# HMS-IDAC/UnMicst

Measured on AMD Instinct MI355X. Metric: tiles/sec (256x256x2) whole-slide inference, higher is better.
Workload: dtype f16x3, cross terms of the layers at <= 1/4 resolution as block-scaled fp6 (MX e2m3) MFMA products; fp32 accumulate

## Files before the change

### unmicst_amd/csrc/umx_conv_f16.hip

```cpp
#include <type_traits>

#include "umx_kernels.h"

namespace umx {

typedef _Float16 h8 __attribute__((ext_vector_type(8)));
typedef float f32x4 __attribute__((ext_vector_type(4)));

template <int I> struct IC { static constexpr int value = I; };
template <int B, int E, typename F>
__device__ __forceinline__ void static_for(F&& f) {
    if constexpr (B < E) {
        f(IC<B>{});
        static_for<B + 1, E>(f);
    }
}

#define UMX_GLDS16(gptr, lptr)                                                                        \
    __builtin_amdgcn_global_load_lds((const __attribute__((address_space(1))) void*)(gptr),           \
                                     (__attribute__((address_space(3))) void*)(lptr), 16, 0, 0)

typedef int i32x6 __attribute__((ext_vector_type(6)));
typedef int i32x8 __attribute__((ext_vector_type(8)));
typedef _Float16 h32 __attribute__((ext_vector_type(32)));

typedef unsigned u32x16 __attribute__((ext_vector_type(16)));
#define UMX_MAX3(dst, a, b, c) asm volatile("v_pk_maximum3_f16 %0, %1, %2, %3" : "=v"(dst) : "v"(a), "v"(b), "v"(c))
#define UMX_MAX3N(dst, a, b, c) asm volatile("v_pk_maximum3_f16 %0, %1, %2, %3 neg_lo:[1,1,1] neg_hi:[1,1,1]" : "=v"(dst) : "v"(a), "v"(b), "v"(c))
#define UMX_MAX3N2(dst, a, b, c) asm volatile("v_pk_maximum3_f16 %0, %1, %2, %3 neg_lo:[0,0,1] neg_hi:[0,0,1]" : "=v"(dst) : "v"(a), "v"(b), "v"(c))
template <int NB>
__device__ __forceinline__ void quant_blocks_e2m3(const h8 (&v)[NB][4], i32x6 (&out)[NB], int (&scale_e8m0)[NB]) {
    h32 x[NB];
    u32x16 d[NB];
#pragma unroll
    for (int b = 0; b < NB; ++b) {
#pragma unroll
        for (int p = 0; p < 4; ++p)
#pragma unroll
            for (int j = 0; j < 8; ++j) x[b][8 * p + j] = v[b][p][j];
        d[b] = __builtin_bit_cast(u32x16, x[b]);
    }
    unsigned P[NB][5], N[NB][5];
#pragma unroll
    for (int t = 0; t < 5; ++t)
#pragma unroll
        for (int b = 0; b < NB; ++b) {
            UMX_MAX3(P[b][t], d[b][3 * t], d[b][3 * t + 1], d[b][3 * t + 2]);
            UMX_MAX3N(N[b][t], d[b][3 * t], d[b][3 * t + 1], d[b][3 * t + 2]);
        }
    unsigned P2[NB][2], N2[NB][2], m2[NB];
#pragma unroll
    for (int b = 0; b < NB; ++b) {
        UMX_MAX3(P2[b][0], P[b][0], P[b][1], P[b][2]);
        UMX_MAX3(N2[b][0], N[b][0], N[b][1], N[b][2]);
    }
#pragma unroll
    for (int b = 0; b < NB; ++b) {
        UMX_MAX3(P2[b][1], P[b][3], P[b][4], d[b][15]);
        UMX_MAX3N2(N2[b][1], N[b][3], N[b][4], d[b][15]);
    }
#pragma unroll
    for (int b = 0; b < NB; ++b) UMX_MAX3(m2[b], P2[b][0], P2[b][1], N2[b][0]);
#pragma unroll
    for (int b = 0; b < NB; ++b) UMX_MAX3(m2[b], m2[b], N2[b][1], N2[b][1]);
#pragma unroll
    for (int b = 0; b < NB; ++b) {
        const unsigned m = m2[b] & 0x7fff7fffu;
        const unsigned mm = max(m & 0xffffu, m >> 16);
        const unsigned ef = __float_as_uint((float)__builtin_bit_cast(_Float16, (unsigned short)mm)) >> 23;
        const unsigned e = max(ef, 3u) - 2u;
        scale_e8m0[b] = (int)e;
        const float sc = __uint_as_float(e << 23);
        asm volatile("v_cvt_scalef32_pk32_fp6_f16 %0, %1, %2" : "=&v"(out[b]) : "v"(x[b]), "v"(sc));
    }
}
__device__ __forceinline__ void quant_block_e2m3(const h8 (&v)[4], i32x6& out, int& scale_e8m0) {
    h8 vv[1][4] = {{v[0], v[1], v[2], v[3]}};
    i32x6 o[1];
    int s[1];
    quant_blocks_e2m3<1>(vv, o, s);
    out = o[0];
    scale_e8m0 = s[0];
}

constexpr int conv_f16x3_waves(int NT, int KMT, int NPH, int MAXP, bool D2S = false) {
    return NPH != 1 || D2S ? 2 : (NT <= 3 && MAXP == 4) ? 4 : (NT <= 3 || (NT <= 5 && MAXP == 4)) ? 3 : 2;
}
template <int NT, int KMT, int NPH, bool DBG = false, int MAXP = 4, bool PK = false, bool D2S = false, bool F6 = false, bool W2 = F6>
__global__ void __launch_bounds__(F6 ? 512 : 256, conv_f16x3_waves(NT, KMT, NPH, MAXP, D2S)) conv_f16x3(const HConvParams p) {
    static_assert(W2 == F6, "W2 only keeps the instantiation names stable: the two-tile workgroup is the F6 form");
    static_assert(!F6 || (NPH == 1 && !PK && !D2S && !DBG), "the fp6 cross-term form runs on the plain / per-phase kernel (no stamped twin: it spills 426 registers)");
    extern __shared__ __attribute__((aligned(16))) unsigned char smem[];

    const int tid = threadIdx.x;
    const int lane = tid & 63;
    constexpr int kNW = F6 ? 2 * kWaves : kWaves;
    const int wave_all = __builtin_amdgcn_readfirstlane(tid >> 6);
    const int half = F6 ? wave_all >> 2 : 0;
    const int wave = F6 ? wave_all & 3 : wave_all;
    const int q = lane >> 4;
    const int li = lane & 15;

    const int TWm = 1 << p.twm_log2, TH = 1 << p.th_log2;
    int bid = blockIdx.x, nblk_i = blockIdx.y, z_i = NPH == 1 ? blockIdx.z : 0;
    if (p.xcd_order == 2) {
        const int YZ = p.nblocks * (NPH == 1 ? p.nphase : 1);
        const int xcd = bid & 7, idx = bid >> 3;
        const int tl = idx / YZ, yz = idx - tl * YZ;
        const int q8 = p.ntiles_grid >> 3, r8 = p.ntiles_grid & 7;
        bid = xcd < r8 ? xcd * (q8 + 1) + tl : r8 * (q8 + 1) + (xcd - r8) * q8 + tl;
        nblk_i = yz % p.nblocks;
        z_i = yz / p.nblocks;
        if (tl >= (xcd < r8 ? q8 + 1 : q8)) return;
    } else if (p.xcd_order) {
        const int nb = gridDim.x, q8 = nb >> 3, r8 = nb & 7, xcd = bid & 7, idx = bid >> 3;
        bid = xcd < r8 ? xcd * (q8 + 1) + idx : r8 * (q8 + 1) + (xcd - r8) * q8 + idx;
    }
    if constexpr (F6) bid = 2 * bid + half;
    const int tx_i = bid % p.tiles_x; bid /= p.tiles_x;
    const int ty_i = bid % p.tiles_y; bid /= p.tiles_y;
    const int img0 = min(bid * p.imgs, p.B);
    const int y0 = ty_i * TH, x0 = tx_i * TWm;
    const HPhase& ph = p.ph[z_i];
    int ph_stage0 = ph.stage0, ph_nstages = ph.nstages;
    size_t split_off = 0;
    if (p.ksplit > 1) {
        const int ks = nblk_i / p.nblocks;
        nblk_i -= ks * p.nblocks;
        ph_stage0 += p.ks0[z_i][ks];
        ph_nstages = p.ks0[z_i][ks + 1] - p.ks0[z_i][ks];
        split_off = (size_t)ks * p.split_stride;
    }
    const int nblk = nblk_i;
    long long t_in = 0, t_wait = 0, t_comp = 0, t_a = 0, t_b = 0, t_vm = 0, t_iss = 0;
    if (DBG && p.dbg) t_in = __builtin_amdgcn_s_memtime();
    int abase[KMT];
#pragma unroll
    for (int m = 0; m < KMT; ++m) {
        const int t = wave * KMT + m;
        const int ig = t >> p.th_log2, ty = t & (TH - 1);
        abase[m] = ((ig * p.nimg_m + (li >> p.twm_log2)) * p.imgplane + ty * p.hw + (li & (TWm - 1))) * p.pix_bytes;
    }

    f32x4 accs[NPH][KMT][NT];
#pragma unroll
    for (int h = 0; h < NPH; ++h)
#pragma unroll
        for (int m = 0; m < KMT; ++m)
#pragma unroll
            for (int n = 0; n < NT; ++n) accs[h][m][n] = (f32x4){0.f, 0.f, 0.f, 0.f};

    const int lo_off = p.lo_off;
    unsigned char* const smem_h = smem + half * p.b_off;
    unsigned char* const Bl = smem + (F6 ? 2 : 1) * p.b_off;
    const uint4* const wbase = ph.w + (size_t)nblk * ph.wblk_stride;

    const int pl = (lane * p.inv_oc_q16) >> 16;
    const int kq = lane - pl * p.OC;
    int pix[MAXP];
#pragma unroll
    for (int j = 0; j < MAXP; ++j) {
        const int px = (wave + kWaves * j) * p.PP + pl;
        int v = -1;
        if (lane < p.nact && px < p.nhalo) {
            const int il = (int)(((float)px + 0.5f) * p.inv_imgplane);
            const int r = px - il * p.imgplane;
            const int hy = (int)(((float)r + 0.5f) * p.inv_hw);
            const int hx = r - hy * p.hw;
            const int gy = y0 + p.ymin + hy, gx = x0 + p.xmin + hx;
            const bool inside = img0 + il < p.B && gy >= 0 && gy < p.H && gx >= 0 && gx < p.W;
            v = inside ? (il * p.H + gy) * p.W + gx : -2;
        }
        pix[j] = v;
    }
    const size_t img_elems = (size_t)p.H * p.W;
    auto act_rsrc = [&](const _Float16* base, int Cs) {
        const size_t left = (size_t)(p.B - img0) * img_elems * Cs * 2;
        return __builtin_amdgcn_make_buffer_rsrc((void*)(base + (size_t)img0 * img_elems * Cs), 0,
                                                 (int)(left < 0x7fffffffu ? left : 0x7fffffffu), 0x00020000);
    };
    const __amdgpu_buffer_rsrc_t r0h = act_rsrc(p.src_hi[0], p.Cs[0]), r0l = act_rsrc(p.src_lo[0], p.Cs[0]);
    const __amdgpu_buffer_rsrc_t r1h = act_rsrc(p.src_hi[1] ? p.src_hi[1] : p.src_hi[0], p.Cs[1]),
                                 r1l = act_rsrc(p.src_lo[1] ? p.src_lo[1] : p.src_lo[0], p.Cs[1]);
    const __amdgpu_buffer_rsrc_t rw =
        __builtin_amdgcn_make_buffer_rsrc((void*)wbase, 0, ph.wblk_stride * 16, 0x00020000);
    const int lane16 = lane * 16;
#define UMX_BLDS16(rsrc, lptr, voff, soff) \
    __builtin_amdgcn_raw_ptr_buffer_load_lds(rsrc, (__attribute__((address_space(3))) void*)(lptr), 16, voff, soff, 0, 0)

    const int kqB0 = kq * p.srcB[0], kqB1 = kq * p.srcB[1];
    auto issue_halo = [&](const HStage& st) {
        const bool g1 = st.group > 0;
        const int pixA = p.srcA[g1 ? 1 : 0];
        const int kqB = g1 ? kqB1 : kqB0;
        const __amdgpu_buffer_rsrc_t rh = g1 ? r1h : r0h, rl = g1 ? r1l : r0l;
        unsigned char* const slot = smem_h + st.plane0 * p.slot_bytes;
        const int soff = st.oct0 * p.srcB[g1 ? 1 : 0];
        const bool kok = kq < st.noct;
#pragma unroll
        for (int j = 0; j < MAXP; ++j) {
            const int i = wave + kWaves * j;
            if (i >= p.ninst) break;
            int pj = pix[j];
            asm volatile("" : "+v"(pj));
            if (pj != -1 && kok) {
                const int voff = pj >= 0 ? (int)__umul24(pj, pixA) + kqB : 0x7fffffff;
                UMX_BLDS16(rh, slot + i * p.piece_bytes, voff, soff);
                UMX_BLDS16(rl, slot + lo_off + i * p.piece_bytes, voff, soff);
            }
        }
    };
    int wq_np = 0, wq_soff = 0;
    unsigned char* wq_dst = Bl;
    const int wq_w = wave_all * 1024;
    auto wq_begin = [&](const HStage& st, int buf) {
        unsigned char* const wl = Bl + buf * p.wbuf_bytes;
        if (wave_all == kNW - 1 && lane < 4) UMX_BLDS16(rw, wl, lane16, st.woff * 16);
        wq_np = F6 ? NT * 4096 : st.nk * (NT * 2048);
        wq_soff = st.woff * 16 + 64;
        wq_dst = wl + 64;
    };
    auto wq_one = [&](int c) {
        const int pc = wq_w + c * (kNW * 1024);
        if (pc < wq_np) UMX_BLDS16(rw, wq_dst + pc, lane16, wq_soff + pc);
    };
    auto wq_drain = [&](int c0) {
        for (int pc = wq_w + c0 * (kNW * 1024); pc < wq_np; pc += kNW * 1024)
            UMX_BLDS16(rw, wq_dst + pc, lane16, wq_soff + pc);
    };

    const int ec_units = (p.head_K > 0 ? (4 + p.head_K) * (NT * 4) + 4 : NT * 16) + (D2S ? 16 : 0);
    auto issue_econst = [&](int buf) {
        if (wave_all == kNW - 1) {
            float* const dst = reinterpret_cast<float*>(Bl + buf * p.wbuf_bytes);
#pragma unroll
            for (int i = 0; i < (8 * NT * 4 + 4 + 63) / 64; ++i)
                if (i * 64 + lane < ec_units)
                    UMX_GLDS16(p.econst + (size_t)nblk * ec_units + i * 64 + lane, dst + i * 256);
        }
    };
    auto issue_app = [&](int buf) {
        if constexpr (D2S) {
            if (p.app_c != nullptr && p.d2s_mix && wave == kWaves - 2) {
                const int apb = 4 * p.app_cw;
                const size_t oHW = (size_t)p.outH * p.outW, left = (size_t)(p.B - img0) * oHW * apb;
                const __amdgpu_buffer_rsrc_t ra = __builtin_amdgcn_make_buffer_rsrc(
                    (void*)(p.app_c + (size_t)img0 * oHW * apb), 0, (int)(left < 0x7fffffffu ? left : 0x7fffffffu), 0x00020000);
                unsigned char* const dst = Bl + buf * p.wbuf_bytes + ec_units * 16;
                const int oy = (lane >> 4) & 1, seg = lane & 15;
#pragma unroll
                for (int i = 0; i < kMW / 2; ++i) {
                    const int t = 2 * i + (lane >> 5);
                    const int irel = (t >> p.th_log2) * p.nimg_m, yt = y0 + (t & (TH - 1));
                    const bool ok = img0 + irel < p.B && seg * 16 < 32 * apb;
                    const int voff = ok ? (int)((irel * (int)oHW + (2 * yt + oy) * p.outW + 2 * x0) * apb + seg * 16) : 0x7fffffff;
                    UMX_BLDS16(ra, dst + i * 1024, voff, 0);
                }
            }
        }
    };
    const int par0 = (ph_nstages + 1) & 1;
    const float* const ec = reinterpret_cast<const float*>(Bl + p.wbuf_bytes);
    if (ph_nstages == 0) { issue_econst(1); issue_app(1); }
    typedef unsigned u32x4 __attribute__((ext_vector_type(4)));
    static_assert(sizeof(HStage) == 16, "one stage = one 16-byte scalar load");
    auto load_stage = [&](int idx) {
        const u32x4 raw = ((const __attribute__((address_space(4))) u32x4*)(unsigned long long)p.stages)[idx];
        HStage st;
        __builtin_memcpy(&st, &raw, sizeof(st));
        return st;
    };
    HStage cur = load_stage(ph_stage0);
    if (ph_nstages > 0) {
        if (cur.group >= 0) issue_halo(cur);
        wq_begin(cur, par0);
        wq_drain(0);
    }
    long long t_pro = 0;
    if (DBG && p.dbg) { t_pro = __builtin_amdgcn_s_memtime(); t_a = t_pro; }
    auto stage_body = [&](const int s) {
        const HStage nxt = load_stage(ph_stage0 + (s + 1 < ph_nstages ? s + 1 : s));
        asm volatile("s_waitcnt vmcnt(0)" ::: "memory");
        if (DBG && p.dbg) { const long long t_v = __builtin_amdgcn_s_memtime(); t_vm += t_v - t_a; }
        __syncthreads();
        if (DBG && p.dbg) { t_b = __builtin_amdgcn_s_memtime(); t_wait += t_b - t_a; }
        if (s + 1 < ph_nstages) {
            if (nxt.group >= 0) issue_halo(nxt);
            wq_begin(nxt, (s + 1 + par0) & 1);
        } else {
            wq_np = 0;
            issue_econst(1);
            issue_app(1);
        }
        if (DBG && p.dbg) t_iss += (long long)__builtin_amdgcn_s_memtime() - t_b;

        const unsigned char* const wl = Bl + ((s + par0) & 1) * p.wbuf_bytes;
        const int cur_nk = F6 ? (cur.nk & 0xff) : cur.nk;
        unsigned kbs[kStageK];
#pragma unroll
        for (int j = 0; j < (F6 ? 2 : kStageK); ++j)
            kbs[j] = (unsigned)*reinterpret_cast<const unsigned short*>(wl + (j * 4 + q) * 2) << 4;
        auto kstep = [&](int h, int j, bool sk) {
            constexpr int kLo = NT / 2, kHi = 2 * (NT / 2);
            constexpr int kImg = F6 ? 1024 : 2048;
            auto live = [&](int n) { return !(D2S && sk && n >= kLo && n < kHi); };
            const unsigned char* const bp = wl + 64 + j * (NT * kImg) + lane * 16;
            const unsigned char* const ap = smem_h + kbs[j];
            h8 ah[KMT], al[KMT];
#pragma unroll
            for (int m = 0; m < KMT; ++m) {
                ah[m] = *reinterpret_cast<const h8*>(ap + abase[m]);
                if constexpr (!F6) al[m] = *reinterpret_cast<const h8*>(ap + abase[m] + lo_off);
            }
            constexpr int kBPre = 2;
            h8 bhq[kBPre + 1], blq[kBPre + 1];
#pragma unroll
            for (int n = 0; n < kBPre && n < NT; ++n) {
                if (!live(n)) continue;
                bhq[n] = *reinterpret_cast<const h8*>(bp + n * kImg);
                if constexpr (!F6) blq[n] = *reinterpret_cast<const h8*>(bp + n * kImg + 1024);
            }
#pragma unroll
            for (int n = 0; n < NT; ++n) {
                wq_one(j * NT + n);
                __builtin_amdgcn_iglp_opt(0);
                if (n + kBPre < NT && live(n + kBPre)) {
                    bhq[(n + kBPre) % (kBPre + 1)] = *reinterpret_cast<const h8*>(bp + (n + kBPre) * kImg);
                    if constexpr (!F6) blq[(n + kBPre) % (kBPre + 1)] = *reinterpret_cast<const h8*>(bp + (n + kBPre) * kImg + 1024);
                }
                if (!live(n)) continue;
                const h8 bh = bhq[n % (kBPre + 1)];
#pragma unroll
                for (int m = 0; m < KMT; ++m) {
                    f32x4 c = accs[h][m][n];
                    if constexpr (!F6) {
                        const h8 bl = blq[n % (kBPre + 1)];
                        c = __builtin_amdgcn_mfma_f32_16x16x32_f16(bh, al[m], c, 0, 0, 0);
                        if (!(PK && n == NT - 1)) c = __builtin_amdgcn_mfma_f32_16x16x32_f16(bl, ah[m], c, 0, 0, 0);
                    }
                    accs[h][m][n] = __builtin_amdgcn_mfma_f32_16x16x32_f16(bh, ah[m], c, 0, 0, 0);
                }
            }
        };
        auto f6step = [&]() {
            if constexpr (F6) {
                const uint2 km = *reinterpret_cast<const uint2*>(wl + (q & 1) * 8);
                const unsigned pl = (q >> 1) ? (unsigned)lo_off : 0u;
                const unsigned ko[4] = {((km.x & 0xffffu) << 4) + pl, ((km.x >> 16) << 4) + pl, ((km.y & 0xffffu) << 4) + pl, ((km.y >> 16) << 4) + pl};
                i32x6 xb[KMT];
                int sx[KMT];
                const unsigned char* const bpq = wl + 64 + 2 * NT * 1024 + lane * 16;
                uint4 w0q[3];
                uint4 w1q[3];
#pragma unroll
                for (int n = 0; n < 2 && n < NT; ++n) {
                    w0q[n] = *reinterpret_cast<const uint4*>(bpq + n * 2048);
                    w1q[n] = *reinterpret_cast<const uint4*>(bpq + n * 2048 + 1024);
                }
#pragma unroll
                for (int m = 0; m < KMT; m += 2) {
                    h8 v[2][4];
#pragma unroll
                    for (int b = 0; b < 2; ++b)
#pragma unroll
                        for (int t = 0; t < 4; ++t) v[b][t] = *reinterpret_cast<const h8*>(smem_h + ko[t] + abase[m + b]);
                    i32x6 o[2];
                    int sc2[2];
                    quant_blocks_e2m3<2>(v, o, sc2);
                    xb[m] = o[0]; xb[m + 1] = o[1];
                    sx[m] = sc2[0]; sx[m + 1] = sc2[1];
                    __builtin_amdgcn_sched_barrier(0);
                }
                const unsigned char* const bp = bpq;
                constexpr int kBPre = 2;
#pragma unroll
                for (int n = 0; n < NT; ++n) {
                    wq_one(2 * NT + n);
                    if (n + kBPre < NT) {
                        w0q[(n + kBPre) % (kBPre + 1)] = *reinterpret_cast<const uint4*>(bp + (n + kBPre) * 2048);
                        w1q[(n + kBPre) % (kBPre + 1)] = *reinterpret_cast<const uint4*>(bp + (n + kBPre) * 2048 + 1024);
                    }
                    const uint4 w0 = w0q[n % (kBPre + 1)], w1 = w1q[n % (kBPre + 1)];
                    const i32x6 wa = (i32x6){(int)w0.x, (int)w0.y, (int)w0.z, (int)w0.w, (int)w1.x, (int)w1.y};
                    const int sa = (int)w1.z;
#pragma unroll
                    for (int m = 0; m < KMT; ++m)
                        if (m == 0)
                            asm volatile("s_nop 1\n\tv_mfma_scale_f32_16x16x128_f8f6f4 %0, %1, %2, %0, %3, %4 op_sel_hi:[0,0,0] cbsz:2 blgp:2"
                                         : "+v"(accs[0][m][n]) : "v"(wa), "v"(xb[m]), "v"(sa), "v"(sx[m]));
                        else
                            asm volatile("v_mfma_scale_f32_16x16x128_f8f6f4 %0, %1, %2, %0, %3, %4 op_sel_hi:[0,0,0] cbsz:2 blgp:2"
                                         : "+v"(accs[0][m][n]) : "v"(wa), "v"(xb[m]), "v"(sa), "v"(sx[m]));
                    __builtin_amdgcn_sched_barrier(0);
                }
            }
        };
        unsigned skips = 0u;
        if constexpr (D2S) skips = __builtin_amdgcn_readfirstlane(*reinterpret_cast<const unsigned*>(wl + 32));
#pragma unroll
        for (int h = 0; h < NPH; ++h) {
            if (NPH > 1 && cur.phase != h) continue;
#pragma unroll
            for (int j = 0; j < (F6 ? 2 : kStageK); ++j) {
                if (j >= cur_nk) break;
                kstep(h, j, D2S && ((skips >> (8 * j)) & 1u) != 0u);
            }
        }
        f6step();
        wq_drain(F6 ? 3 * NT : cur_nk * NT);
        cur = nxt;
        if (DBG && p.dbg) { t_a = __builtin_amdgcn_s_memtime(); t_comp += t_a - t_b; }
    };
    for (int s = 0; s < ph_nstages; ++s) stage_body(s);
    auto pk_sum = [](float v) {
        const unsigned u = __float_as_uint(v);
        const auto sw = __builtin_amdgcn_permlane32_swap(u, u, false, false);
        return __uint_as_float(sw[0]) + __uint_as_float(sw[1]);
    };
    if constexpr (PK && NPH == 1) {
#pragma unroll
        for (int m = 0; m < KMT; ++m)
#pragma unroll
            for (int r = 0; r < 4; ++r) accs[0][m][NT - 1][r] = pk_sum(accs[0][m][NT - 1][r]);
    }
    struct DbgOut {
        const HConvParams& p; long long t_in, t_pro, t_wait, t_comp, t_epi; int tid; const long long& t_vm; const long long& t_iss;
        __device__ ~DbgOut() {
            if (DBG && p.dbg && tid == 0) {
                const long long t_end = __builtin_amdgcn_s_memtime();
                const size_t w = ((size_t)blockIdx.z * gridDim.y + blockIdx.y) * gridDim.x + blockIdx.x;
                long long* d = p.dbg + w * 7;
                d[0] = t_pro - t_in; d[1] = t_wait; d[2] = t_comp; d[3] = t_end - t_epi; d[4] = t_end - t_in; d[5] = t_vm; d[6] = t_iss;
            }
        }
    } dbg_out{p, t_in, t_pro, t_wait, t_comp, DBG && p.dbg ? (long long)__builtin_amdgcn_s_memtime() : 0, tid, t_vm, t_iss};

    asm volatile("s_waitcnt vmcnt(0)" ::: "memory");
    __syncthreads();
    const float4* const ec4 = reinterpret_cast<const float4*>(ec);


    unsigned vmax = 0u;
    const float slope = p.act == ACT_RELU ? 0.f : p.act == ACT_LEAKY ? kLeakySlope : 1.f;
    auto arith_v = [&](const f32x4 (&A)[NT], float (&out)[NT][4], auto POST, auto TRACK) {
        constexpr bool post = decltype(POST)::value, track = decltype(TRACK)::value;
        if constexpr (post) asm volatile("; epilogue arithmetic, second affine");
        else asm volatile("; epilogue arithmetic");
        float dyn = 1.f;
        if constexpr (!track) dyn = (p.dyn[0] ? *p.dyn[0] : 1.f) * (p.dyn[1] ? *p.dyn[1] : 1.f);
#pragma unroll
        for (int n = 0; n < NT; ++n) {
            const float4 ps = ec4[0 * NT * 4 + n * 4 + q], pb = ec4[1 * NT * 4 + n * 4 + q];
            float psa[4] = {ps.x, ps.y, ps.z, ps.w};
            const float pba[4] = {pb.x, pb.y, pb.z, pb.w};
            if constexpr (!track) {
#pragma unroll
                for (int r = 0; r < 4; ++r) psa[r] *= dyn;
            }
            float qsa[4] = {1.f, 1.f, 1.f, 1.f}, qba[4] = {0.f, 0.f, 0.f, 0.f};
            if constexpr (post) {
                const float4 qs = ec4[2 * NT * 4 + n * 4 + q], qb = ec4[3 * NT * 4 + n * 4 + q];
                qsa[0] = qs.x; qsa[1] = qs.y; qsa[2] = qs.z; qsa[3] = qs.w;
                qba[0] = qb.x; qba[1] = qb.y; qba[2] = qb.z; qba[3] = qb.w;
            }
#pragma unroll
            for (int r = 0; r < 4; ++r) {
                float v = A[n][r] * psa[r] + pba[r];
                v = __builtin_amdgcn_fmed3f(v, v * slope, INFINITY);
                if constexpr (post) v = v * qsa[r] + qba[r];
                if constexpr (track) vmax = max(vmax, __float_as_uint(v) & 0x7fffffffu);
                out[n][r] = v;
            }
            __builtin_amdgcn_sched_barrier(0);
        }
    };
    auto arith = [&](const f32x4 (&A)[NT], float (&out)[NT][4], auto TRACK) {
        if (p.post_affine) arith_v(A, out, std::true_type{}, TRACK);
        else arith_v(A, out, std::false_type{}, TRACK);
    };
    constexpr std::true_type kTrack{};
    constexpr std::false_type kNoTrack{};

    if constexpr (NPH == 1) {
        if (p.head_K > 0) {
            const int K = p.head_K;
            constexpr int NS2 = (NT + 1) / 2;
            const float* const hsb = ec + (4 + K) * (NT * 16);
            typedef unsigned u32x4 __attribute__((ext_vector_type(4)));
            u32x4 Hh[NS2], Hl[NS2];
#pragma unroll
            for (int s2 = 0; s2 < NS2; ++s2) {
                Hh[s2] = *reinterpret_cast<const u32x4*>(p.head_frag + (s2 * 2 + 0) * 64 + lane);
                Hl[s2] = *reinterpret_cast<const u32x4*>(p.head_frag + (s2 * 2 + 1) * 64 + lane);
            }
            f32x4 lg = (f32x4){0.f, 0.f, 0.f, 0.f};
            static_for<0, KMT>([&](auto MC) {
                constexpr int m = decltype(MC)::value;
                float res[NT][4];
                arith(accs[0][m], res, kTrack);
#pragma unroll
                for (int s2 = 0; s2 < NS2; ++s2) {
                    h8 bh, bl;
#pragma unroll
                    for (int j = 0; j < 8; ++j) {
                        const int nt = 2 * s2 + (j >> 2);
                        const float t = nt < NT ? res[nt < NT ? nt : 0][j & 3] : 0.f;
                        bh[j] = (_Float16)t;
                        bl[j] = (_Float16)(t - (float)bh[j]);
                    }
                    u32x4 ah = Hh[s2], al = Hl[s2];
                    if constexpr ((m & 3) != 0) {
                        constexpr int ctrl = 0x110 + 4 * (m & 3);
#pragma unroll
                        for (int d = 0; d < 4; ++d) {
                            ah[d] = (unsigned)__builtin_amdgcn_update_dpp(0, (int)ah[d], ctrl, 0xF, 0xF, true);
                            al[d] = (unsigned)__builtin_amdgcn_update_dpp(0, (int)al[d], ctrl, 0xF, 0xF, true);
                        }
                    }
                    const h8 wh = __builtin_bit_cast(h8, ah), wl = __builtin_bit_cast(h8, al);
                    lg = __builtin_amdgcn_mfma_f32_16x16x32_f16(wh, bl, lg, 0, 0, 0);
                    lg = __builtin_amdgcn_mfma_f32_16x16x32_f16(wl, bh, lg, 0, 0, 0);
                    lg = __builtin_amdgcn_mfma_f32_16x16x32_f16(wh, bh, lg, 0, 0, 0);
                }
                if ((m & 3) == 3 || m == KMT - 1) {
                    const int mq = (m & ~3) + q;
                    const int t = wave * KMT + mq;
                    const int ig = t >> p.th_log2, ty = t & (TH - 1);
                    const int img = img0 + ig * p.nimg_m + (li >> p.twm_log2);
                    if (mq < KMT && img < p.B) {
                        float e[4], mx = -INFINITY;
#pragma unroll
                        for (int k = 0; k < 4; ++k) {
                            e[k] = k < K ? lg[k] * hsb[k] + hsb[8 + k] : -INFINITY;
                            mx = fmaxf(mx, e[k]);
                        }
                        float sum = 0.f;
#pragma unroll
                        for (int k = 0; k < 4; ++k) {
                            e[k] = __expf(e[k] - mx);
                            sum += e[k];
                        }
                        const float inv = __builtin_amdgcn_rcpf(sum);
                        float* const d = p.probs + ((long)(img * p.outH + y0 + ty) * p.outW + x0 + (li & (TWm - 1))) * K;
                        if (K == 3) {
                            struct __attribute__((packed, aligned(4))) F3 { float a, b, c; };
                            *reinterpret_cast<F3*>(d) = F3{e[0] * inv, e[1] * inv, e[2] * inv};
                        } else {
#pragma unroll
                            for (int k = 0; k < 4; ++k)
                                if (k < K) d[k] = e[k] * inv;
                        }
                    }
                    lg = (f32x4){0.f, 0.f, 0.f, 0.f};
                }
            });
            if (vmax >= 0x476a6000u) atomicOr(p.overflow_flag, 1);
            return;
        }
        if (p.dst_f32) {
#pragma unroll
            for (int m = 0; m < KMT; ++m) {
                const int t = wave * KMT + m;
                const int ig = t >> p.th_log2, ty = t & (TH - 1);
                const int img = img0 + ig * p.nimg_m + (li >> p.twm_log2);
                float res[NT][4];
                arith(accs[0][m], res, kNoTrack);
                if (img >= p.B) continue;
                const long pix = (long)(img * p.outH + (y0 + ty) * p.o_mul + ph.oy_off) * p.outW +
                                 (x0 + (li & (TWm - 1))) * p.o_mul + ph.ox_off;
#pragma unroll
                for (int n = 0; n < NT; ++n) {
                    const int c0 = nblk * (NT * 16) + n * 16 + 4 * q;
                    const float* const v = res[n];
                    float* const d = p.dst_f32 + split_off + pix * p.Cout + c0;
                    if ((p.Cout & 3) == 0) {
                        if (c0 < p.Cout) *reinterpret_cast<float4*>(d) = make_float4(v[0], v[1], v[2], v[3]);
                    } else {
#pragma unroll
                        for (int r = 0; r < 4; ++r)
                            if (c0 + r < p.Cout) d[r] = v[r];
                    }
                }
            }
            return;
        }
    }

    const bool dpl = p.dst_planar != 0;
    const int dImg = p.Cds * p.outH * p.outW;
    const int dPix = dpl ? 8 : p.Cds;
    const int dOct = dpl ? p.outH * p.outW * 8 : 8;
    const int noct = p.Cds >> 3;
    const int oct_q = q >> 1;
    const bool setB = (q & 1) != 0;
    unsigned char* const bhi = reinterpret_cast<unsigned char*>(p.dst_hi + (size_t)img0 * dImg);
    unsigned char* const blo = reinterpret_cast<unsigned char*>(p.dst_lo + (size_t)img0 * dImg);
    typedef _Float16 h2 __attribute__((ext_vector_type(2)));
    auto pack_split = [](float v0, float v1, unsigned& hw, unsigned& lw) {
        h2 h, l;
        h[0] = (_Float16)v0; h[1] = (_Float16)v1;
        l[0] = (_Float16)(v0 - (float)h[0]); l[1] = (_Float16)(v1 - (float)h[1]);
        hw = __builtin_bit_cast(unsigned, h);
        lw = __builtin_bit_cast(unsigned, l);
    };
    struct EC { float ps[4], pb[4], qs[4], qb[4]; };
    auto load_ec = [&](int n, auto POST) {
        EC e;
        const float4 ps = ec4[0 * NT * 4 + n * 4 + q], pb = ec4[1 * NT * 4 + n * 4 + q];
        e.ps[0] = ps.x; e.ps[1] = ps.y; e.ps[2] = ps.z; e.ps[3] = ps.w;
        e.pb[0] = pb.x; e.pb[1] = pb.y; e.pb[2] = pb.z; e.pb[3] = pb.w;
        if constexpr (decltype(POST)::value) {
            const float4 qs = ec4[2 * NT * 4 + n * 4 + q], qb = ec4[3 * NT * 4 + n * 4 + q];
            e.qs[0] = qs.x; e.qs[1] = qs.y; e.qs[2] = qs.z; e.qs[3] = qs.w;
            e.qb[0] = qb.x; e.qb[1] = qb.y; e.qb[2] = qb.z; e.qb[3] = qb.w;
        }
        return e;
    };
    auto act1 = [&](float a, const EC& e, int r, auto POST) {
        float v = a * e.ps[r] + e.pb[r];
        v = __builtin_amdgcn_fmed3f(v, v * slope, INFINITY);
        if constexpr (decltype(POST)::value) v = v * e.qs[r] + e.qb[r];
        return v;
    };
    constexpr bool kApp = NT <= 5;
    const bool lane_app = kApp && p.app_c != nullptr && oct_q == (p.app_oct & 1) && (p.app_oct >> 1) >= nblk * NT &&
                          (p.app_oct >> 1) < (nblk + 1) * NT;
    auto app_load = [&](int apix, unsigned& ah, unsigned& al) {
        ah = al = 0u;
        if (lane_app && apix >= 0) {
            const size_t px = (size_t)img0 * p.outH * p.outW + apix;
            if (p.app_cw == 2) {
                const uint2 w = *reinterpret_cast<const uint2*>(p.app_c + px * 8);
                ah = w.x; al = w.y;
            } else {
                const unsigned w = *reinterpret_cast<const unsigned*>(p.app_c + px * 4);
                ah = w & 0xffffu; al = w >> 16;
            }
        }
    };
    auto store_unit = [&](int n, const float (&a)[4], const float (&b)[4], int off, bool ok, int apix, unsigned app_h, unsigned app_l) {
        const int oct_u = (nblk * NT + n) * 2 + oct_q;
        const bool app = kApp && lane_app && apix >= 0 && oct_u == p.app_oct;
#pragma unroll
        for (int r = 0; r < 4; ++r)
            vmax = max(vmax, max(__float_as_uint(a[r]) & 0x7fffffffu, __float_as_uint(b[r]) & 0x7fffffffu));
        unsigned ah0, ah1, al0, al1, bh0, bh1, bl0, bl1;
        pack_split(a[0], a[1], ah0, al0);
        pack_split(a[2], a[3], ah1, al1);
        pack_split(b[0], b[1], bh0, bl0);
        pack_split(b[2], b[3], bh1, bl1);
        const auto h0 = __builtin_amdgcn_permlane16_swap(ah0, bh0, false, false);
        const auto h1 = __builtin_amdgcn_permlane16_swap(ah1, bh1, false, false);
        const auto l0 = __builtin_amdgcn_permlane16_swap(al0, bl0, false, false);
        const auto l1 = __builtin_amdgcn_permlane16_swap(al1, bl1, false, false);
        const int oct = oct_u;
        if (ok && oct < noct) {
            const unsigned o = (unsigned)(off + oct * dOct) * 2u;
            uint4 uh = make_uint4(h0[0], h1[0], h0[1], h1[1]), ul = make_uint4(l0[0], l1[0], l0[1], l1[1]);
            if (app) {
                if (p.app_word == 1) { uh.y = app_h; ul.y = app_l; }
                else if (p.app_word == 2) { uh.z = app_h; ul.z = app_l; }
                else { uh.w = app_h; ul.w = app_l; }
            }
            *reinterpret_cast<uint4*>(bhi + o) = uh;
            *reinterpret_cast<uint4*>(blo + o) = ul;
        }
    };
    auto emit_t = [&](const f32x4 (&A)[NT], const f32x4 (&B)[NT], int off, bool ok, int apix, unsigned app_h, unsigned app_l, auto POST) {
        if constexpr (decltype(POST)::value) asm volatile("; epilogue stores, second affine");
        else asm volatile("; epilogue stores");
#pragma unroll
        for (int n = 0; n < NT; ++n) {
            const EC e = load_ec(n, POST);
            float a[4], b[4];
#pragma unroll
            for (int r = 0; r < 4; ++r) {
                float av = A[n][r], bv = B[n][r];
                if constexpr (PK && NPH == 4) {
                    if (n == NT - 1) { av = pk_sum(av); bv = pk_sum(bv); }
                }
                a[r] = act1(av, e, r, POST); b[r] = act1(bv, e, r, POST);
            }
            store_unit(n, a, b, off, ok, apix, app_h, app_l);
            __builtin_amdgcn_sched_barrier(0);
        }
    };
    auto emit = [&](const f32x4 (&A)[NT], const f32x4 (&B)[NT], int off, bool ok, int apix, unsigned app_h, unsigned app_l) {
        if (p.post_affine) emit_t(A, B, off, ok, apix, app_h, app_l, std::true_type{});
        else emit_t(A, B, off, ok, apix, app_h, app_l, std::false_type{});
    };
    auto emit_pool_t = [&](const f32x4 (&R0)[NT], const f32x4 (&R1)[NT], const f32x4 (&R2)[NT], const f32x4 (&R3)[NT], int off,
                           bool ok, auto POST) {
        if constexpr (decltype(POST)::value) asm volatile("; pooled epilogue stores, second affine");
        else asm volatile("; pooled epilogue stores");
#pragma unroll
        for (int n = 0; n < NT; ++n) {
            const EC e = load_ec(n, POST);
            float a[4], b[4];
#pragma unroll
            for (int r = 0; r < 4; ++r) {
                const float va = fmaxf(act1(R0[n][r], e, r, POST), act1(R1[n][r], e, r, POST));
                const float vb = fmaxf(act1(R2[n][r], e, r, POST), act1(R3[n][r], e, r, POST));
                const float sa = __builtin_bit_cast(
                    float, __builtin_amdgcn_update_dpp(0, __builtin_bit_cast(int, va), 0xB1 , 0xF, 0xF, false));
                const float sb = __builtin_bit_cast(
                    float, __builtin_amdgcn_update_dpp(0, __builtin_bit_cast(int, vb), 0xB1, 0xF, 0xF, false));
                a[r] = fmaxf(va, sa);
                b[r] = fmaxf(vb, sb);
            }
            store_unit(n, a, b, off, ok, -1, 0u, 0u);
            __builtin_amdgcn_sched_barrier(0);
        }
    };
    const int dImgPix = p.outH * p.outW;
    int app_img = 0;
    auto pix_off = [&](int t, int i, int& y_tile, int& x_tile) {
        const int ig = t >> p.th_log2;
        y_tile = y0 + (t & (TH - 1));
        x_tile = x0 + (i & (TWm - 1));
        const int irel = ig * p.nimg_m + (i >> p.twm_log2);
        if constexpr (kApp) app_img = irel * dImgPix;
        return img0 + irel < p.B ? irel * dImg : -1;
    };
    if constexpr (D2S) {
        static_assert(NPH == 1 && (KMT & 1) == 0 && !PK, "the depth-to-space form runs on the plain kernel");
        const int z = z_i;
        const int* const dtab = reinterpret_cast<const int*>(ec) + 4 * NT * 16 + z * (2 * NT + 8);
        const bool mix = p.d2s_mix != 0;
        constexpr int NTR = NT - 1;
        const int rowB = 2 * p.outW * dPix;
#pragma unroll
        for (int m = 0; m < KMT; m += 2) {
            int yt, xt;
            const int ib = pix_off(wave * KMT + m, li, yt, xt);
            const int off = ib + ((yt * 2) * p.outW + xt * 2) * dPix + (setB ? rowB : 0);
            const bool ok = ib >= 0;
            auto body = [&](auto POST) {
#pragma unroll
                for (int n = 0; n < NT; ++n) {
                    if (n == NTR && mix) break;
                    const EC e = load_ec(n, POST);
                    float a[4], b[4];
#pragma unroll
                    for (int r = 0; r < 4; ++r) { a[r] = act1(accs[0][m][n][r], e, r, POST); b[r] = act1(accs[0][m + 1][n][r], e, r, POST); }
#pragma unroll
                    for (int r = 0; r < 4; ++r)
                        vmax = max(vmax, max(__float_as_uint(a[r]) & 0x7fffffffu, __float_as_uint(b[r]) & 0x7fffffffu));
                    unsigned ah0, ah1, al0, al1, bh0, bh1, bl0, bl1;
                    pack_split(a[0], a[1], ah0, al0);
                    pack_split(a[2], a[3], ah1, al1);
                    pack_split(b[0], b[1], bh0, bl0);
                    pack_split(b[2], b[3], bh1, bl1);
                    const auto h0 = __builtin_amdgcn_permlane16_swap(ah0, bh0, false, false);
                    const auto h1 = __builtin_amdgcn_permlane16_swap(ah1, bh1, false, false);
                    const auto l0 = __builtin_amdgcn_permlane16_swap(al0, bl0, false, false);
                    const auto l1 = __builtin_amdgcn_permlane16_swap(al1, bl1, false, false);
                    const int dsel = dtab[2 * n + oct_q];
                    if (ok && dsel >= 0) {
                        const unsigned o = (unsigned)(off + dsel) * 2u;
                        *reinterpret_cast<uint4*>(bhi + o) = make_uint4(h0[0], h1[0], h0[1], h1[1]);
                        *reinterpret_cast<uint4*>(blo + o) = make_uint4(l0[0], l1[0], l0[1], l1[1]);
                    }
                    __builtin_amdgcn_sched_barrier(0);
                }
            };
            if (p.post_affine) body(std::true_type{});
            else body(std::false_type{});
        }
        if (mix) {
            const int dmix = dtab[2 * NT + q];
            const int cmix = dtab[2 * NT + 4 + q];
            const bool app_on = p.app_c != nullptr;
            const int apb = 4 * p.app_cw;
            const unsigned char* const apl = reinterpret_cast<const unsigned char*>(ec) + ec_units * 16 + (cmix >> 1) * 256 +
                                             (2 * li + (cmix & 1)) * apb;
            auto tail = [&](auto POST) {
                const EC e = load_ec(NTR, POST);
#pragma unroll
                for (int m = 0; m < KMT; ++m) {
                    int yt, xt;
                    const int ib = pix_off(wave * KMT + m, li, yt, xt);
                    float a[4];
#pragma unroll
                    for (int r = 0; r < 4; ++r) {
                        a[r] = act1(accs[0][m][NTR][r], e, r, POST);
                        vmax = max(vmax, __float_as_uint(a[r]) & 0x7fffffffu);
                    }
                    uint4 uh = make_uint4(0u, 0u, 0u, 0u), ul = make_uint4(0u, 0u, 0u, 0u);
                    pack_split(a[0], a[1], uh.x, ul.x);
                    pack_split(a[2], a[3], uh.y, ul.y);
                    if (app_on && dmix >= 0) {
                        unsigned aph, apl_w;
                        const unsigned char* const src = apl + (wave * KMT + m) * 512;
                        if (p.app_cw == 2) {
                            const uint2 w = *reinterpret_cast<const uint2*>(src);
                            aph = w.x; apl_w = w.y;
                        } else {
                            const unsigned w = *reinterpret_cast<const unsigned*>(src);
                            aph = w & 0xffffu; apl_w = w >> 16;
                        }
                        if (p.app_word == 1) { uh.y = aph; ul.y = apl_w; }
                        else if (p.app_word == 2) { uh.z = aph; ul.z = apl_w; }
                        else { uh.w = aph; ul.w = apl_w; }
                    }
                    if (ib >= 0 && dmix >= 0) {
                        const unsigned o = (unsigned)(ib + ((yt * 2) * p.outW + xt * 2) * dPix + dmix) * 2u;
                        *reinterpret_cast<uint4*>(bhi + o) = uh;
                        *reinterpret_cast<uint4*>(blo + o) = ul;
                    }
                    __builtin_amdgcn_sched_barrier(0);
                }
            };
            if (p.post_affine) tail(std::true_type{});
            else tail(std::false_type{});
        } else {
#pragma unroll
            for (int m = 0; m < KMT; m += 2) {
                int yt, xt;
                const int ib = pix_off(wave * KMT + m, li, yt, xt);
                const int off = ib + ((yt * 2) * p.outW + xt * 2) * dPix + (setB ? rowB : 0);
                auto last = [&](auto POST) {
                    const EC e = load_ec(NTR, POST);
                    float a[4], b[4];
#pragma unroll
                    for (int r = 0; r < 4; ++r) { a[r] = act1(accs[0][m][NTR][r], e, r, POST); b[r] = act1(accs[0][m + 1][NTR][r], e, r, POST); }
#pragma unroll
                    for (int r = 0; r < 4; ++r)
                        vmax = max(vmax, max(__float_as_uint(a[r]) & 0x7fffffffu, __float_as_uint(b[r]) & 0x7fffffffu));
                    unsigned ah0, ah1, al0, al1, bh0, bh1, bl0, bl1;
                    pack_split(a[0], a[1], ah0, al0);
                    pack_split(a[2], a[3], ah1, al1);
                    pack_split(b[0], b[1], bh0, bl0);
                    pack_split(b[2], b[3], bh1, bl1);
                    const auto h0 = __builtin_amdgcn_permlane16_swap(ah0, bh0, false, false);
                    const auto h1 = __builtin_amdgcn_permlane16_swap(ah1, bh1, false, false);
                    const auto l0 = __builtin_amdgcn_permlane16_swap(al0, bl0, false, false);
                    const auto l1 = __builtin_amdgcn_permlane16_swap(al1, bl1, false, false);
                    const int dsel = dtab[2 * NTR + oct_q];
                    if (ib >= 0 && dsel >= 0) {
                        const unsigned o = (unsigned)(off + dsel) * 2u;
                        *reinterpret_cast<uint4*>(bhi + o) = make_uint4(h0[0], h1[0], h0[1], h1[1]);
                        *reinterpret_cast<uint4*>(blo + o) = make_uint4(l0[0], l1[0], l0[1], l1[1]);
                    }
                };
                if (p.post_affine) last(std::true_type{});
                else last(std::false_type{});
            }
        }
    } else if constexpr (NPH == 4) {
        int ibs[KMT], pixs[KMT][2], apx[KMT][2];
        unsigned aph[KMT][2], apl[KMT][2];
#pragma unroll
        for (int m = 0; m < KMT; ++m) {
            int yt, xt;
            ibs[m] = pix_off(wave * KMT + m, li, yt, xt);
#pragma unroll
            for (int pu = 0; pu < 2; ++pu) {
                pixs[m][pu] = (yt * 2 + pu) * p.outW + xt * 2 + (setB ? 1 : 0);
                apx[m][pu] = ibs[m] >= 0 ? app_img + pixs[m][pu] : -1;
                app_load(apx[m][pu], aph[m][pu], apl[m][pu]);
            }
        }
#pragma unroll
        for (int m = 0; m < KMT; ++m)
#pragma unroll
            for (int pu = 0; pu < 2; ++pu)
                emit(accs[pu * 2 + 0][m], accs[pu * 2 + 1][m], ibs[m] + pixs[m][pu] * dPix, ibs[m] >= 0, apx[m][pu], aph[m][pu], apl[m][pu]);
    } else if (p.pool) {
        static_assert(NPH == 4 || KMT == 4, "the pooled epilogue pairs the two pooled rows of a wave");
        int yt, xt;
        const int ib = pix_off(wave * KMT + (setB ? 2 : 0), li, yt, xt);
        const int off = ib + ((yt >> 1) * p.outW + (xt >> 1)) * dPix;
        const bool ok = ib >= 0 && (li & 1) == 0;
        if (p.post_affine) emit_pool_t(accs[0][0], accs[0][1], accs[0][2], accs[0][3], off, ok, std::true_type{});
        else emit_pool_t(accs[0][0], accs[0][1], accs[0][2], accs[0][3], off, ok, std::false_type{});
    } else {
        static_assert((KMT & 1) == 0, "M-tiles are stored in pairs");
        const int om = p.o_mul;
#pragma unroll
        for (int m = 0; m < KMT; m += 2) {
            int yt, xt;
            const int ib = pix_off(wave * KMT + m + (setB ? 1 : 0), li, yt, xt);
            const int pix = (yt * om + ph.oy_off) * p.outW + xt * om + ph.ox_off;
            const int apix = ib >= 0 ? app_img + pix : -1;
            unsigned ah, al;
            app_load(apix, ah, al);
            emit(accs[0][m], accs[0][m + 1], ib + pix * dPix, ib >= 0, apix, ah, al);
        }
    }
    if (vmax >= 0x476a6000u) atomicOr(p.overflow_flag, 1);
}

template <int NT, int KMT, int NPH, bool DBG, int MAXP, bool PK = false, bool D2S = false, bool F6 = false>
static hipError_t launch_h_k(const HConvParams& p, hipStream_t stream) {
    const int img_groups = (p.B + p.imgs - 1) / p.imgs;
    dim3 grid((unsigned)(img_groups * p.tiles_y * p.tiles_x), (unsigned)p.nblocks, (unsigned)(NPH == 1 ? p.nphase : 1));
    if (F6) {
        if (p.xcd_order == 2 || p.ksplit > 1) return hipErrorInvalidValue;
        grid.x = (grid.x + 1) / 2;
    }
    if (p.ksplit > 1) {
        if (p.xcd_order == 2 || !p.dst_f32 || p.head_K > 0 || p.ksplit > kMaxKSplit) return hipErrorInvalidValue;
        grid.y *= (unsigned)p.ksplit;
    }
    if (p.xcd_order == 2) {
        if (p.ntiles_grid != (int)grid.x || p.tiles_per_xcd * 8 < p.ntiles_grid) return hipErrorInvalidValue;
        grid = dim3((unsigned)(8 * p.tiles_per_xcd) * grid.y * grid.z, 1, 1);
    }
    const size_t lds = (size_t)p.lds_bytes;
    const void* kern = reinterpret_cast<const void*>(conv_f16x3<NT, KMT, NPH, DBG, MAXP, PK, D2S, F6>);
    if (lds > 48 * 1024) {
        hipError_t e = hipFuncSetAttribute(kern, hipFuncAttributeMaxDynamicSharedMemorySize, (int)lds);
        if (e != hipSuccess) return e;
    }
    hipLaunchKernelGGL((conv_f16x3<NT, KMT, NPH, DBG, MAXP, PK, D2S, F6>), grid, dim3(F6 ? 512 : 256), lds, stream, p);
    return hipGetLastError();
}

template <int NT, int KMT, int NPH>
static hipError_t launch_h_nt(const HConvParams& p, hipStream_t stream) {
    constexpr bool has4 = true, has12 = NT <= 5 && !(NPH == 4 && NT > 3);
    if (p.maxp != 4 && p.maxp != 12) return hipErrorInvalidValue;
    if (p.f6) {
        if constexpr (NT == 9 && NPH == 1) {
            if (p.maxp == 4 && !p.pk && !p.d2s && !p.dbg) return launch_h_k<NT, KMT, NPH, false, 4, false, false, true>(p, stream);
        }
        return hipErrorInvalidValue;
    }
    if (p.d2s) {
        if constexpr (NT >= 5 && NPH == 1) {
            if constexpr (NT == 9) {
                if (p.maxp == 4 && !p.pk && p.dbg) return launch_h_k<NT, KMT, NPH, true, 4, false, true>(p, stream);
            }
            if (p.maxp == 4 && !p.pk) return launch_h_k<NT, KMT, NPH, false, 4, false, true>(p, stream);
        }
        return hipErrorInvalidValue;
    }
    if (p.pk) {
        if constexpr (NT >= 2 && NT <= 5) {
            if constexpr (has12) {
                if (p.maxp == 12) return launch_h_k<NT, KMT, NPH, false, 12, true>(p, stream);
            }
            if (p.maxp == 4) return launch_h_k<NT, KMT, NPH, false, 4, true>(p, stream);
        }
        return hipErrorInvalidValue;
    }
    if constexpr (has12) {
        if (p.maxp == 12) {
            if constexpr (NT == 3 && NPH == 4) {
                if (p.dbg) return launch_h_k<NT, KMT, NPH, true, 12>(p, stream);
            }
            return launch_h_k<NT, KMT, NPH, false, 12>(p, stream);
        }
    }
    if constexpr (has4) {
        if (p.maxp == 4) {
            if constexpr ((NT == 3 || NT == 5 || NT == 9) && !(NPH == 4 && NT == 3)) {
                if (p.dbg) return launch_h_k<NT, KMT, NPH, true, 4>(p, stream);
            }
            return launch_h_k<NT, KMT, NPH, false, 4>(p, stream);
        }
    }
    return hipErrorInvalidValue;
}

hipError_t launch_conv_f16(const HConvParams& p, hipStream_t stream) {
    if (p.fused_phases) {
        switch (p.NT) {
            case 1: return launch_h_nt<1, 2, 4>(p, stream);
            case 2: return launch_h_nt<2, 2, 4>(p, stream);
            case 3: return launch_h_nt<3, 2, 4>(p, stream);
            case 4: return launch_h_nt<4, 2, 4>(p, stream);
            case 5: return launch_h_nt<5, 2, 4>(p, stream);
            default: return hipErrorInvalidValue;
        }
    }
    switch (p.NT) {
        case 1: return launch_h_nt<1, kMT, 1>(p, stream);
        case 2: return launch_h_nt<2, kMT, 1>(p, stream);
        case 3: return launch_h_nt<3, kMT, 1>(p, stream);
        case 4: return launch_h_nt<4, kMT, 1>(p, stream);
        case 5: return launch_h_nt<5, kMT, 1>(p, stream);
        case 6: return launch_h_nt<6, kMT, 1>(p, stream);
        case 7: return launch_h_nt<7, kMT, 1>(p, stream);
        case 8: return launch_h_nt<8, kMT, 1>(p, stream);
        case 9: return launch_h_nt<9, kMT, 1>(p, stream);
        default: return hipErrorInvalidValue;
    }
}

__global__ void __launch_bounds__(256) split_f32_kernel(const float* __restrict__ x, size_t npix, int C, int Cs, float scale,
                                                       _Float16* __restrict__ hi, _Float16* __restrict__ lo) {
    const size_t total = npix * (size_t)Cs;
    for (size_t e = (size_t)blockIdx.x * blockDim.x + threadIdx.x; e < total; e += (size_t)gridDim.x * blockDim.x) {
        const size_t px = e / Cs;
        const int c = (int)(e - px * Cs);
        const float v = c < C ? x[px * C + c] * scale : 0.f;
        const _Float16 h = (_Float16)v;
        hi[e] = h;
        lo[e] = (_Float16)(v - (float)h);
    }
}
template <int CW>
__global__ void __launch_bounds__(256) split_f32_compact_kernel(const float* __restrict__ x, size_t npix, int C, float scale,
                                                               _Float16* __restrict__ out) {
    for (size_t px = (size_t)blockIdx.x * blockDim.x + threadIdx.x; px < npix; px += (size_t)gridDim.x * blockDim.x) {
        _Float16 w[2 * CW];
#pragma unroll
        for (int c = 0; c < CW; ++c) {
            const float v = c < C ? x[px * C + c] * scale : 0.f;
            w[c] = (_Float16)v;
            w[CW + c] = (_Float16)(v - (float)w[c]);
        }
#pragma unroll
        for (int c = 0; c < 2 * CW; ++c) out[px * (2 * CW) + c] = w[c];
    }
}

hipError_t launch_split_f32(const float* x, size_t npix, int C, int Cs, float scale, _Float16* hi, _Float16* lo, int cw,
                            hipStream_t stream) {
    if (npix == 0) return hipSuccess;
    if (cw > 0) {
        const unsigned blocks = (unsigned)((npix + 255) / 256 < 256 * 16 ? (npix + 255) / 256 : 256 * 16);
        if (cw == 1) hipLaunchKernelGGL(split_f32_compact_kernel<1>, dim3(blocks), dim3(256), 0, stream, x, npix, C, scale, hi);
        else if (cw == 2) hipLaunchKernelGGL(split_f32_compact_kernel<2>, dim3(blocks), dim3(256), 0, stream, x, npix, C, scale, hi);
        else if (cw == 4) hipLaunchKernelGGL(split_f32_compact_kernel<4>, dim3(blocks), dim3(256), 0, stream, x, npix, C, scale, hi);
        else return hipErrorInvalidValue;
        return hipGetLastError();
    }
    const size_t total = npix * (size_t)Cs;
    const unsigned blocks = (unsigned)((total + 255) / 256 < 256 * 16 ? (total + 255) / 256 : 256 * 16);
    hipLaunchKernelGGL(split_f32_kernel, dim3(blocks), dim3(256), 0, stream, x, npix, C, Cs, scale, hi, lo);
    return hipGetLastError();
}

template <int CW, int SRC>
__global__ void __launch_bounds__(256) gather_split_kernel(const void* __restrict__ image_v, double inv_max, int C_img, int band_row0,
                                                          int band_rows, TileGeom g, int Cn, double mean, double stdv,
                                                          int tile0, int ntiles, float scale, uint4* __restrict__ hi,
                                                          uint4* __restrict__ lo, const unsigned* __restrict__ mm) {
    constexpr int NC = CW > 0 ? CW : 8;
    const size_t total = (size_t)ntiles * g.P * g.P;
    double rlo[NC], rhi[NC];
    if constexpr (SRC != 0) {
#pragma unroll
        for (int c = 0; c < NC; ++c) {
            const int pl = C_img == 1 ? 0 : (c < Cn ? c : 0);
            rlo[c] = mm ? __dmul_rn((double)mm[16 * pl], inv_max) : 0.0;
            rhi[c] = mm ? __dmul_rn((double)mm[16 * pl + 1], inv_max) : 0.0;
        }
    }
    for (size_t e = (size_t)blockIdx.x * blockDim.x + threadIdx.x; e < total; e += (size_t)gridDim.x * blockDim.x) {
        const int x = (int)(e % g.P);
        const size_t r1 = e / g.P;
        const int y = (int)(r1 % g.P);
        const int t = tile0 + (int)(r1 / g.P);
        const int pr = t / g.npc, pc = t - pr * g.npc;
        const int iy = pr * g.sub + y - g.margin, ix = pc * g.sub + x - g.margin;
        const bool inside = iy >= 0 && iy < g.H && ix >= 0 && ix < g.W;
        union { _Float16 h[8]; uint4 u; uint2 u2; unsigned u1; } vh, vl;
        vh.u = make_uint4(0, 0, 0, 0);
        vl.u = make_uint4(0, 0, 0, 0);
#pragma unroll
        for (int c = 0; c < NC; ++c) {
            float f = 0.f;
            if (c < Cn) {
                double v = 0.0;
                if (inside) {
                    const size_t at = ((size_t)(C_img == 1 ? 0 : c) * band_rows + (iy - band_row0)) * g.W + ix;
                    if constexpr (SRC == 0) v = static_cast<const double*>(image_v)[at];
                    else if constexpr (SRC == 1) v = __dmul_rn((double)static_cast<const unsigned short*>(image_v)[at], inv_max);
                    else v = __dmul_rn((double)static_cast<const unsigned char*>(image_v)[at], inv_max);
                    if constexpr (SRC != 0) {
                        if (mm) {
                            if (rlo[c] != rhi[c]) v = __dmul_rn(__ddiv_rn(__dsub_rn(v, rlo[c]), __dsub_rn(rhi[c], rlo[c])), 0.983);
                            else v = fmin(fmax(v, 0.0), 0.983);
                        }
                    }
                }
                f = (float)((v - mean) / stdv) * scale;
            }
            vh.h[c] = (_Float16)f;
            vl.h[c] = (_Float16)(f - (float)vh.h[c]);
        }
        if constexpr (CW == 0) {
            hi[e] = vh.u;
            lo[e] = vl.u;
        } else if constexpr (CW == 1) {
            reinterpret_cast<unsigned*>(hi)[e] = (vh.u1 & 0xffffu) | (vl.u1 << 16);
        } else if constexpr (CW == 2) {
            reinterpret_cast<uint2*>(hi)[e] = make_uint2(vh.u1, vl.u1);
        } else {
            hi[e] = make_uint4(vh.u2.x, vh.u2.y, vl.u2.x, vl.u2.y);
        }
    }
}

hipError_t launch_gather_split(const void* image, int raw_bits, int C_img, int band_row0, int band_rows, const TileGeom& g, int Cn,
                               double mean, double stdv, int tile0, int ntiles, float scale, _Float16* hi, _Float16* lo, int cw,
                               hipStream_t stream, const unsigned* mm) {
    if (ntiles <= 0) return hipSuccess;
    if (mm && raw_bits == 0) return hipErrorInvalidValue;
    if (Cn > 8 || (cw > 0 && Cn > cw) || (raw_bits != 0 && raw_bits != 8 && raw_bits != 16)) return hipErrorInvalidValue;
    const size_t total = (size_t)ntiles * g.P * g.P;
    const unsigned blocks = (unsigned)((total + 255) / 256 < 256 * 16 ? (total + 255) / 256 : 256 * 16);
    uint4* const h4 = reinterpret_cast<uint4*>(hi);
    uint4* const l4 = reinterpret_cast<uint4*>(lo);
    const double inv_max = raw_bits == 16 ? 1.0 / 65535 : 1.0 / 255;
#define UMX_GS2(CWV, SRCV) hipLaunchKernelGGL((gather_split_kernel<CWV, SRCV>), dim3(blocks), dim3(256), 0, stream, image, inv_max, C_img, \
                                              band_row0, band_rows, g, Cn, mean, stdv, tile0, ntiles, scale, h4, l4, mm)
#define UMX_GS(CWV) do { if (raw_bits == 0) UMX_GS2(CWV, 0); else if (raw_bits == 16) UMX_GS2(CWV, 1); else UMX_GS2(CWV, 2); } while (0)
    if (cw == 0) UMX_GS(0);
    else if (cw == 1) UMX_GS(1);
    else if (cw == 2) UMX_GS(2);
    else if (cw == 4) UMX_GS(4);
    else return hipErrorInvalidValue;
#undef UMX_GS
#undef UMX_GS2
    return hipGetLastError();
}

}
```

Baseline: 21120.

## Spread next-stage halo loads across MFMA k-step slots instead of issuing in bulk

When NPH==1 and NT>=5, the halo loads for the next stage are no longer issued all at once right after the barrier. Each per-wave halo piece now takes one slot in the per-n load schedule ahead of the weight-queue loads, so global-to-LDS traffic is interleaved with MFMA work rather than bunched up. Drain logic is extended to cover slots that were not consumed, including F6 stages with fewer k-steps. This adds index bookkeeping and branches inside the hot loop, and it reorders halo loads relative to weight loads.

```diff
diff --git a/unmicst_amd/csrc/umx_conv_f16.hip b/unmicst_amd/csrc/umx_conv_f16.hip
--- a/unmicst_amd/csrc/umx_conv_f16.hip
+++ b/unmicst_amd/csrc/umx_conv_f16.hip
@@ -228,6 +228,49 @@
         for (int pc = wq_w + c0 * (kNW * 1024); pc < wq_np; pc += kNW * 1024)
             UMX_BLDS16(rw, wq_dst + pc, lane16, wq_soff + pc);
     };
+    constexpr bool kSpread = NPH == 1 && NT >= 5;
+    static_assert(!F6 || NT >= 2 * MAXP, "F6 form: the halo slots lie in the stage's first k-step, the only one every stage has");
+    HStage hq_st = {};
+    int hq_np = 0;
+    auto hq_begin = [&](const HStage& st) {
+        hq_st = st;
+        hq_np = st.group >= 0 ? 2 * min((p.ninst - wave + kWaves - 1) / kWaves, MAXP) : 0;
+    };
+    auto hq_one = [&](int c) {
+        const int j = c >> 1;
+        const bool g1 = hq_st.group > 0, lo = (c & 1) != 0;
+        const int i = wave + kWaves * j;
+        int pj = pix[j];
+        asm volatile("" : "+v"(pj));
+        if (pj != -1 && kq < hq_st.noct) {
+            const int voff = pj >= 0 ? (int)__umul24(pj, p.srcA[g1 ? 1 : 0]) + (g1 ? kqB1 : kqB0) : 0x7fffffff;
+            unsigned char* const dst = smem_h + hq_st.plane0 * p.slot_bytes + (lo ? lo_off : 0) + i * p.piece_bytes;
+            UMX_BLDS16(lo ? (g1 ? r1l : r0l) : (g1 ? r1h : r0h), dst, voff, hq_st.oct0 * p.srcB[g1 ? 1 : 0]);
+        }
+    };
+    auto ld_one = [&](int c) {
+        if constexpr (kSpread) {
+            if (c < 2 * MAXP && c < hq_np) hq_one(c);
+            else wq_one(c - hq_np);
+        } else {
+            wq_one(c);
+        }
+    };
+    auto ld_drain = [&](int c0, int c1) {
+        if constexpr (kSpread) {
+            if constexpr (NT < 2 * MAXP) {
+#pragma unroll
+                for (int c = NT; c < 2 * MAXP; ++c)
+                    if (c >= c0 && c < hq_np) hq_one(c);
+            }
+            const int k0 = max(c0 - hq_np, 0);
+            if (c1 < 0) wq_drain(k0);
+            else
+                for (int k = k0; k < c1 - hq_np; ++k) wq_one(k);
+        } else {
+            wq_drain(c0);
+        }
+    };
 
     const int ec_units = (p.head_K > 0 ? (4 + p.head_K) * (NT * 4) + 4 : NT * 16) + (D2S ? 16 : 0);
     auto issue_econst = [&](int buf) {
@@ -285,10 +328,12 @@
         __syncthreads();
         if (DBG && p.dbg) { t_b = __builtin_amdgcn_s_memtime(); t_wait += t_b - t_a; }
         if (s + 1 < ph_nstages) {
-            if (nxt.group >= 0) issue_halo(nxt);
+            if constexpr (kSpread) hq_begin(nxt);
+            else if (nxt.group >= 0) issue_halo(nxt);
             wq_begin(nxt, (s + 1 + par0) & 1);
         } else {
             wq_np = 0;
+            hq_np = 0;
             issue_econst(1);
             issue_app(1);
         }
@@ -322,7 +367,7 @@
             }
 #pragma unroll
             for (int n = 0; n < NT; ++n) {
-                wq_one(j * NT + n);
+                ld_one(j * NT + n);
                 __builtin_amdgcn_iglp_opt(0);
                 if (n + kBPre < NT && live(n + kBPre)) {
                     bhq[(n + kBPre) % (kBPre + 1)] = *reinterpret_cast<const h8*>(bp + (n + kBPre) * kImg);
@@ -375,7 +420,7 @@
                 constexpr int kBPre = 2;
 #pragma unroll
                 for (int n = 0; n < NT; ++n) {
-                    wq_one(2 * NT + n);
+                    ld_one(2 * NT + n);
                     if (n + kBPre < NT) {
                         w0q[(n + kBPre) % (kBPre + 1)] = *reinterpret_cast<const uint4*>(bp + (n + kBPre) * 2048);
                         w1q[(n + kBPre) % (kBPre + 1)] = *reinterpret_cast<const uint4*>(bp + (n + kBPre) * 2048 + 1024);
@@ -406,8 +451,9 @@
                 kstep(h, j, D2S && ((skips >> (8 * j)) & 1u) != 0u);
             }
         }
+        if (F6 && cur_nk < 2) ld_drain(NT, 2 * NT);
         f6step();
-        wq_drain(F6 ? 3 * NT : cur_nk * NT);
+        ld_drain(F6 ? 3 * NT : cur_nk * NT, -1);
         cur = nxt;
         if (DBG && p.dbg) { t_a = __builtin_amdgcn_s_memtime(); t_comp += t_a - t_b; }
     };
```

Measured after the change: 19930. 5.6% lower.
